# Opendigitalradio/ODR-AudioEnc

Measured on AMD Instinct MI355X. Metric: real-time stereo DAB MP2 streams sustained (frames/s) @128 kbps/48 kHz, higher is better.
Workload: dtype f64; 1 GPU; 4096 streams/GPU x 48 kHz stereo (mode 's') x 128 kbps, psy 1, full encode (BASELINE configs[1]), 32 frames/stream/step; streams_per_gpu=4096, parallelism=streams sharded over 1 GPU(s), no data-path collective

## Files before the change

### odr-audioenc_amd/csrc/mp2_fb.h

```cpp
#ifndef MP2_WAVE_PARTS
#error "include mp2_wave.h"
#endif
TL_FN void tl_filterbank(TlMainLds &w, const TlBlockShared *TL_RESTRICT B, const double *TL_RESTRICT enw_s, const int nch, PARGA(double, smp, 36))
{
    constexpr int FB = TlMainLds::kFbBatch;
        PA(int, xa, 16); PA(int, xb, 16);
        TL_LANES_BEGIN
        const int c = lane & 1, i = lane >> 1;
        const int ya = i == 0 ? 16 : i + 16, yb = i == 0 ? 16 : (i <= 16 ? 16 - i : 80 - i);
        for (int b = 0; b < 2; b++)
            for (int j = 1; j < 8; j++) {
                L(xa)[8 * b + ((0 - j) & 7)] = c < nch ? w.u.fbk.pcm[c][TL_HIST + 32 * b + 31 - ya - 64 * j] : 0;
                L(xb)[8 * b + ((0 - j) & 7)] = c < nch ? w.u.fbk.pcm[c][TL_HIST + 32 * b + 31 - yb - 64 * j] : 0;
            }
        TL_LANES_END
        TlMainLds::YpRows yp = w.yp;
#pragma unroll
        for (int b0 = 0; b0 < 36; b0 += FB) {
            TL_LANES_BEGIN
            const int c = lane & 1, i = lane >> 1;
            if (c < nch) {
                const int ya = i == 0 ? 16 : i + 16, yb = i == 0 ? 16 : (i <= 16 ? 16 - i : 80 - i);
                const uint64_t keep = i == 0 ? 0ull : ~0ull, flip = (i == 0 || i > 16) ? 0x8000000000000000ull : 0ull;
                int na[FB], nb[FB];
                double cf[8], ta[FB];
#pragma unroll
                for (int bb = 0; bb < FB; bb++) {
                    na[bb] = w.u.fbk.pcm[c][TL_HIST + 32 * (b0 + bb) + 31 - ya];
                    nb[bb] = w.u.fbk.pcm[c][TL_HIST + 32 * (b0 + bb) + 31 - yb];
                }
#pragma unroll
                for (int j = 0; j < 8; j++) cf[j] = enw_s[ya + 64 * j];
#pragma unroll
                for (int bb = 0; bb < FB; bb++) { TL_KEEP(na[bb]); TL_KEEP(nb[bb]); }
#pragma unroll
                for (int bb = 0; bb < FB; bb++) {
                    const int b = b0 + bb, q = 8 * (b & 1), h = b >> 1;
                    L(xa)[q + (h & 7)] = na[bb];
                    double t = (double)L(xa)[q + (h & 7)] * cf[0];
                    for (int j = 1; j < 8; j++) t += (double)L(xa)[q + ((h - j) & 7)] * cf[j];
                    ta[bb] = t;
                }
#pragma unroll
                for (int j = 0; j < 8; j++) cf[j] = enw_s[yb + 64 * j];
#pragma unroll
                for (int bb = 0; bb < FB; bb++) {
                    const int b = b0 + bb, q = 8 * (b & 1), h = b >> 1;
                    L(xb)[q + (h & 7)] = nb[bb];
                    double t = (double)L(xb)[q + (h & 7)] * cf[0];
                    for (int j = 1; j < 8; j++) t += (double)L(xb)[q + ((h - j) & 7)] * cf[j];
                    yp[bb][TL_YP_ROW * (2 * c + (i & 1)) + (i >> 1)] = ta[bb] + tl_u2d((tl_d2u(t) & keep) ^ flip);
                }
            }
            TL_LANES_END
            PA(double, part, FB);
            TL_LANES_BEGIN
            const int c = lane & 1, sb = lane >> 1, par = sb < 16 ? 0 : 1, r = sb < 16 ? sb : 31 - sb;
            double acc[FB];
            for (int bb = 0; bb < FB; bb++) acc[bb] = 0.0;
            if (c < nch)
                for (int k = 0; k < 16; k += 2) {
                    const double m0 = B->dct_t[k][par][r], m1 = B->dct_t[k + 1][par][r];
                    for (int bb = 0; bb < FB; bb++) {
                        double y0, y1;
                        TL_LD2(&yp[bb][TL_YP_ROW * (2 * c + par) + k], y0, y1);
                        acc[bb] += m0 * y0;
                        acc[bb] += m1 * y1;
                    }
                }
            for (int bb = 0; bb < FB; bb++) L(part)[bb] = acc[bb];
            TL_LANES_END
            PA(double, oth, FB);
            TL_MIRROR_SB_F64(oth, part, FB);
            TL_LANES_BEGIN
            const int sb = lane >> 1;
            if (sb < 16) { for (int bb = 0; bb < FB; bb++) L(smp)[b0 + bb] = L(part)[bb] + L(oth)[bb]; }
            else { for (int bb = 0; bb < FB; bb++) L(smp)[b0 + bb] = L(oth)[bb] - L(part)[bb]; }
            TL_LANES_END
        }
}
```

### odr-audioenc_amd/csrc/mp2_pack.h

```cpp
#ifndef MP2_WAVE_PARTS
#error "include mp2_wave.h"
#endif
struct TlFrameOut { uint8_t *bytes; uint32_t *words; uint8_t *scfcrc; };
template <int PSY, int NCH = 0>
TL_FN void tl_encode_frame(TlMainLds &w, const TlTables *TL_RESTRICT T, const TlBlockShared *TL_RESTRICT B,
                           const TlConfig *TL_RESTRICT C, const TlPsyOut *TL_RESTRICT PO,
                           const TlPcmView &pv, int xpad_len, const TlFrameOut &fo,
                           const double *TL_RESTRICT enw_s, const TlPackTables *TL_RESTRICT K, int padding, TlTaps *taps, long long *sp)
{
    constexpr int FB = TlMainLds::kFbBatch;
    const int nch = NCH ? NCH : C->nch, sblimit = C->sblimit;
    PA(double, smp, 36);
    PA(int, scf, 3);

    TL_STAMP(sp, 0);
    TL_PRIO2(TL_PS_FB);
    tl_filterbank(w, B, enw_s, nch, smp);

    TL_STAMP(sp, 1);
    TL_PRIO2(1);
#if !defined(TL_EMULATE) && TL_ENC_LEVEL >= 5
    for (int b = 0; b < 36; b++) TL_KEEP(smp[b]);
    scf[0] = scf[1] = scf[2] = 0;
#endif
    PV(int, a_ln); PV(int, a_nbal);
    TL_LANES_BEGIN
    {
        const int c = lane & 1, sb = lane >> 1;
        const bool live = c < nch && sb < sblimit;
        L(a_ln) = live ? C->line[sb] : 0;
        L(a_nbal) = live ? C->nbal[sb] : 0;
    }
    TL_LANES_END
    TL_LANES_BEGIN
    const int c = lane & 1, sb = lane >> 1;
    if (TL_ENC_LEVEL >= 5) { }
    else if (c < nch && sb < sblimit) {
        unsigned lo = 63;
        for (int gr = 0; gr < 3; gr++) {
            double m = fabs(L(smp)[gr * 12 + 11]);
            for (int j = 10; j >= 0; j--) { double t = fabs(L(smp)[gr * 12 + j]); if (t > m) m = t; }
            unsigned idx = tl_sf_index(B->scalefactor, m);
            L(scf)[gr] = (int)idx;
            w.scf[c][gr][sb] = (uint8_t)idx;
            if (idx < lo) lo = idx;
        }
        w.minidx[c][sb] = (uint8_t)lo;
    } else {
        L(scf)[0] = L(scf)[1] = L(scf)[2] = 0;
        if (sb >= sblimit || c >= nch) { w.minidx[c][sb] = 63; w.scf[c][0][sb] = w.scf[c][1][sb] = w.scf[c][2][sb] = 0; }
    }
    TL_LANES_END

    if (TL_ENC_LEVEL < 5 && C->mode0 == 1) {
        for (int gr = 0; gr < 3; gr++) {
            PV(double, jm);
            TL_LANES_BEGIN L(jm) = 0.0; TL_LANES_END
#pragma unroll
            for (int j = 11; j >= 0; j--) {
                PV(double, other);
                TL_SWAP1_F64(other, , smp, [gr * 12 + j]);
                TL_LANES_BEGIN
                double t = fabs(.5 * (L(smp)[gr * 12 + j] + L(other)));
                if (j == 11 || t > L(jm)) L(jm) = t;
                TL_LANES_END
            }
            TL_LANES_BEGIN
            const int c = lane & 1, sb = lane >> 1;
            if (c == 0 && sb < sblimit) w.jscale[gr][sb] = (uint8_t)tl_sf_index(B->scalefactor, L(jm));
            TL_LANES_END
        }
    }

    if (taps) {
        TL_LANES_BEGIN
        const int c = lane & 1, sb = lane >> 1;
        for (int b = 0; b < 36; b++) taps->sb_sample[c][b / 12][b % 12][sb] = L(smp)[b];
        for (int gr = 0; gr < 3; gr++) { taps->scalar_pre[c][gr][sb] = w.scf[c][gr][sb]; if (c == 0) taps->j_scale[gr][sb] = C->mode0 == 1 && sb < sblimit ? w.jscale[gr][sb] : 0; }
        taps->max_sc[c][sb] = (c < nch && sb < sblimit) ? B->scalefactor[w.minidx[c][sb]] : 1E-20;
        TL_LANES_END
    }

    TL_STAMP(sp, 2);
    if constexpr (TL_ENC_LEVEL >= 5) { }
    else if constexpr (PSY == 0) {
        TL_LANES_BEGIN
        const int c = lane & 1, sb = lane >> 1;
        if (c < nch) {
            int m = sb < sblimit ? (int)w.minidx[c][sb] : 0;
            w.smr[c][sb] = 2.0 * (30.0 - m) - C->p0_athmin[sb];
        }
        TL_LANES_END
    } else if constexpr (PSY == 2) {
        TL_LANES_BEGIN
        const int c = lane & 1, sb = lane >> 1;
        if (c < nch) w.smr[c][sb] = PO->a[c][sb];
        TL_LANES_END
    } else {
        static_assert(PSY == TL_PSY_EXT, "models 1 and 3");
        TL_LANES_BEGIN
        const int c = lane & 1, sb = lane >> 1;
        if (c < nch) {
            const double a = w.smr[c][sb], m = w.psy_m[c][sb];
            const double val = B->scale_db[w.minidx[c][sb]];
            const double top = a > val ? a : val;
            w.smr[c][sb] = top - m;
        }
        TL_LANES_END
    }

    TL_STAMP(sp, 3);
    TL_LANES_BEGIN
    const int c = lane & 1, sb = lane >> 1;
    if (TL_ENC_LEVEL < 5 && c < nch && sb < sblimit) {
        int s0 = L(scf)[0], s1 = L(scf)[1], s2 = L(scf)[2];
        int d0 = s0 - s1, d1 = s1 - s2;
        int c0 = d0 <= -3 ? 0 : d0 < 0 ? 1 : d0 == 0 ? 2 : d0 < 3 ? 3 : 4;
        int c1 = d1 <= -3 ? 0 : d1 < 0 ? 1 : d1 == 0 ? 2 : d1 < 3 ? 3 : 4;
        const unsigned p = B->sfpat[c0 * 5 + c1];
        const int m02 = s0 > s2 ? s2 : s0;
        const unsigned q0 = p & 3u, q1 = (p >> 2) & 3u, q2 = (p >> 4) & 3u;
        const int n0 = q0 == 0 ? s0 : q0 == 1 ? s1 : q0 == 2 ? s2 : m02;
        const int n1 = q1 == 0 ? s0 : q1 == 1 ? s1 : q1 == 2 ? s2 : m02;
        const int n2 = q2 == 0 ? s0 : q2 == 1 ? s1 : q2 == 2 ? s2 : m02;
        const int sel = (int)(p >> 6);
        s0 = n0; s1 = n1; s2 = n2;
        L(scf)[0] = s0; L(scf)[1] = s1; L(scf)[2] = s2;
        w.scf[c][0][sb] = (uint8_t)s0; w.scf[c][1][sb] = (uint8_t)s1; w.scf[c][2][sb] = (uint8_t)s2;
        w.scfsi[c][sb] = (uint8_t)sel;
    } else w.scfsi[c][sb] = 0;
    w.balloc[c][sb] = 0;
    TL_LANES_END

    const int lg_frame = C->frame_bytes + padding;
    int adb = lg_frame * 8 - (C->dab_ext * 8 + (xpad_len ? xpad_len : 2) * 8);
    int mode = C->mode0, mode_ext = C->mode_ext0, jsbound = C->jsbound0;
    PV(int, a_sfs); PV(int, a_sfs_o); PV(double, a_smr); PV(double, a_smr_o);
    TL_LANES_BEGIN
    const int c = lane & 1, sb = lane >> 1;
    const bool live = c < nch && sb < sblimit;
    L(a_sfs) = live ? 6 * tl_sfs_count(w.scfsi[c][sb]) : 0;
    L(a_sfs_o) = (live && nch == 2) ? 6 * tl_sfs_count(w.scfsi[1 - c][sb]) : 0;
    L(a_smr) = live ? w.smr[c][sb] : 0.0;
    L(a_smr_o) = (live && nch == 2) ? w.smr[1 - c][sb] : 0.0;
    TL_LANES_END
    if (TL_ENC_LEVEL < 4 && C->mode0 == 1) {
        PV(int, nz_own); PV(int, nz_jnt);
        TL_LANES_BEGIN
        int bo = 0, bj = 0;
        if (lane < 2 * sblimit) {
            const int ln = L(a_ln), maxAlloc = (1 << L(a_nbal)) - 1;
            double sv[15];
#pragma unroll
            for (int q = 0; q < 15; q++) sv[q] = B->snr_line[ln][q];
            int n1 = 0, n2 = 0;
#pragma unroll
            for (int q = 0; q < 15; q++) {
                const bool inr = q < maxAlloc - 1;
                n1 += (inr && !((sv[q] - L(a_smr)) >= 0.0)) ? 1 : 0;
                n2 += (inr && !((sv[q] - L(a_smr_o)) >= 0.0)) ? 1 : 0;
            }
            n2 = n2 > n1 ? n2 : n1;
            bo = n1 > 0 ? B->bits12_line[ln][n1] + 2 + L(a_sfs) : 0;
            bj = n2 > 0 ? B->bits12_line[ln][n2] + 4 + L(a_sfs) + L(a_sfs_o) : 0;
        }
        L(nz_own) = bo; L(nz_jnt) = bj;
        TL_LANES_END
        mode = 0; mode_ext = 0; jsbound = sblimit;
        int tries = 0, try_ext = 4;
        for (;;) {
// ... 186 lines not shown
                const bool three = L(q_grp) == 3;
                const unsigned M = (unsigned)L(q_steps);
                const unsigned fa = TL_SELECT(three, v[2], v[0]), fc = TL_SELECT(three, v[0], v[2]);
                const unsigned inner = v[1] + M * fc;
                tl_put_bits48(frame, pos, (uint64_t)fa + (uint64_t)M * (uint64_t)inner, L(q_grp) * nb);
            }
            if (taps) for (int x = 0; x < 3; x++) taps->subband[c][gr][j0 + x][sb] = (c < nch) ? v[x] : 0;
            TL_LANES_END
        }
        }
    }

    TL_STAMP(sp, 5);
    TL_PRIO2(1);
    unsigned crc16 = 0;
    if (TL_ENC_LEVEL < 1) {
    {
        const int n = 16 + (p_scf - 48);
        PV(uint32_t, part);
        TL_LANES_BEGIN
        uint32_t acc = 0;
        const bool preset = lane >= 62;
        const int first = 8 * lane;
        if (first < n || preset) {
            const int byte = lane < 2 ? lane + 2 : lane + 4;
            const int cnt = preset ? 8 : (n - first < 8 ? n - first : 8);
            const int e0 = preset ? n + 8 * (63 - lane) : 16 + (n - first - cnt);
            const uint16_t *xt = &K->crc_xpow[e0];
            const unsigned v = preset ? 0xffu : ((frame[byte >> 2] >> (24 - 8 * (byte & 3))) & 0xffu) >> (8 - cnt);
            unsigned x8[8];
#pragma unroll
            for (int k = 0; k < 8; k++) x8[k] = xt[k];
#pragma unroll
            for (int k = 0; k < 8; k++) acc ^= (0u - ((v >> k) & 1u)) & x8[k];
        }
        L(part) = acc;
        TL_LANES_END
        crc16 = TL_WAVE_XOR_U32(part) & 0xffffu;
    }
    const int tail = lg_frame - 2 - C->dab_ext;
    PV(int, rlen); PV(uint32_t, rcrc);
    TL_LANES_BEGIN
    const int c = lane & 1, sb = lane >> 1;
    uint32_t rec = 0;
    if (c < nch && sb < sblimit && w.balloc[c][sb]) {
        const uint32_t s0 = (uint32_t)L(scf)[0] >> 3, s1 = (uint32_t)L(scf)[1] >> 3, s2 = (uint32_t)L(scf)[2] >> 3;
        switch (w.scfsi[c][sb]) {
        case 0: rec = (9u << 16) | (s0 << 6) | (s1 << 3) | s2; break;
        case 1: case 3: rec = (6u << 16) | (s0 << 3) | s2; break;
        default: rec = (3u << 16) | s0; break;
        }
    }
    if (lane == 0) tl_put_bits(frame, 32, crc16, 16);
    L(rlen) = (int)(rec >> 16); L(rcrc) = rec & 0x1ffu;
    TL_LANES_END
    {
        PV(int, lex);
        TL_WAVE_EXSCAN_I32(lex, rlen);
        const int f[5] = {0, 4, 8, 16, 30};
        int gend[4], gfirst[4], glast[4];
        for (int g = 0; g < 4; g++) {
            gfirst[g] = f[g]; glast[g] = f[g + 1] > sblimit ? sblimit : f[g + 1];
            const int e = 2 * glast[g];
            gend[g] = (g < C->dab_ext && glast[g] > gfirst[g]) ? TL_READLANE_I32(lex, e) : 0;
        }
        PV(uint32_t, part); PV(uint32_t, pscan);
        TL_LANES_BEGIN
        const int sb = lane >> 1;
        const int g = sb < 4 ? 0 : sb < 8 ? 1 : sb < 16 ? 2 : 3;
        const int after = (g == 0 ? gend[0] : g == 1 ? gend[1] : g == 2 ? gend[2] : gend[3]) - L(lex) - L(rlen);
        const int e0 = after + 8;
        unsigned xp = K->crc8_xpow[e0 < 0 ? 0 : e0 > 319 ? 319 : e0];
        unsigned acc = 0;
        const unsigned rb = L(rcrc);
#pragma unroll
        for (int b = 0; b < 9; b++) {
            acc ^= ((rb >> b) & 1u) ? xp : 0u;
            xp = ((xp << 1) & 0xffu) ^ ((xp & 0x80u) ? 0x1Du : 0u);
        }
        L(part) = (L(rlen) && sb < sblimit) ? acc : 0u;
        TL_LANES_END
        TL_WAVE_INCL_XSCAN_U32(pscan, part);
        unsigned c8g[4];
        for (int g = 0; g < 4; g++) {
            c8g[g] = 0;
            if (g < C->dab_ext && glast[g] > gfirst[g]) {
                c8g[g] = (unsigned)TL_READLANE_I32(pscan, 2 * glast[g] - 1);
                if (gfirst[g] > 0) c8g[g] ^= (unsigned)TL_READLANE_I32(pscan, 2 * gfirst[g] - 1);
            }
        }
        TL_LANES_BEGIN
        if (lane < C->dab_ext) {
            const int grp = C->dab_ext - 1 - lane;
            const unsigned c8 = (grp == 0 ? c8g[0] : grp == 1 ? c8g[1] : grp == 2 ? c8g[2] : c8g[3]) & 0xffu;
            tl_put_bits(frame, (tail + lane) * 8, c8, 8);
            w.ncentre[lane] = (int16_t)c8;
        }
        TL_LANES_END
    }
    TL_LANES_BEGIN
    if (xpad_len) {
        const int xstart = lg_frame - C->dab_ext - xpad_len;
        for (int i = lane; i < xpad_len; i += 64) {
            int bytepos = i < xpad_len - 2 ? xstart + i : lg_frame - 2 + (i - (xpad_len - 2));
            tl_put_bits(frame, bytepos * 8, w.xpad[i], 8);
        }
    }
    TL_LANES_END

    } else {
        TL_LANES_BEGIN
        if (lane < 4) w.ncentre[lane] = 0;
        TL_LANES_END
    }
    if (taps) {
        TL_LANES_BEGIN
        const int c = lane & 1, sb = lane >> 1;
        taps->smr[c][sb] = (c < nch && (C->psy != 1 || sb < sblimit)) ? w.smr[c][sb] : 0.0;
        taps->scfsi[c][sb] = w.scfsi[c][sb]; taps->bit_alloc[c][sb] = w.balloc[c][sb];
        for (int gr = 0; gr < 3; gr++) taps->scalar[c][gr][sb] = w.scf[c][gr][sb];
        if (lane == 0) { taps->adb_left = adb_left; taps->mode = mode; taps->mode_ext = mode_ext; taps->jsbound = jsbound; taps->crc16 = (int)crc16; }
        if (lane < 4) taps->scfcrc[lane] = lane < C->dab_ext ? (uint8_t)w.ncentre[lane] : 0;
        TL_LANES_END
    }

    TL_STAMP(sp, 6);
    const int nwords = (lg_frame + 3) >> 2;
    TL_LANES_BEGIN
    for (int i = lane; i < nwords; i += 64) {
        if (fo.words) fo.words[i] = frame[i];
        else {
            const uint32_t le = tl_bswap(frame[i]);
            const int rem = lg_frame - 4 * i;
            if (rem >= 4) ((uint32_t *)fo.bytes)[i] = le;
            else for (int b = 0; b < rem; b++) fo.bytes[4 * i + b] = (uint8_t)(le >> (8 * b));
        }
    }
    if (lane < 4) fo.scfcrc[lane] = lane < C->dab_ext ? (uint8_t)w.ncentre[lane] : 0;
    TL_LANES_END
    TL_PRIO2(0);
    TL_STAMP(sp, 7);
}

template <int PSY>
TL_FN void tl_encode_pair(TlMainLds &w, const TlBlockShared *TL_RESTRICT B, const TlConfig *TL_RESTRICT C, const TlPsyOut *const (&PO)[2],
                          const int (&xpad_len)[2], const uint8_t *const (&xpad_src)[2], const TlFrameOut (&fo)[2],
                          const double *TL_RESTRICT enw_s, const TlPackTables *TL_RESTRICT K, const int (&padding)[2])
{
    const int sblimit = C->sblimit;
    const int padpk = padding[0] | (padding[1] << 1);
    PA(double, smp, 36);
    PA(int, scf, 3);
    TL_PRIO2(TL_PS_FB);
    tl_filterbank(w, B, enw_s, 2, smp);
    TL_PRIO2(1);
    TL_LANES_BEGIN
    const int c = lane & 1, sb = lane >> 1;
    if (sb < sblimit) {
        unsigned lo = 63;
        for (int gr = 0; gr < 3; gr++) {
            double m = fabs(L(smp)[gr * 12 + 11]);
            for (int j = 10; j >= 0; j--) { double t = fabs(L(smp)[gr * 12 + j]); if (t > m) m = t; }
            unsigned idx = tl_sf_index(B->scalefactor, m);
            L(scf)[gr] = (int)idx;
            if (idx < lo) lo = idx;
        }
        w.minidx[c][sb] = (uint8_t)lo;
    } else {
        L(scf)[0] = L(scf)[1] = L(scf)[2] = 0;
        w.minidx[c][sb] = 63;
    }
    TL_LANES_END
    TL_LANES_BEGIN
    const int c = lane & 1, sb = lane >> 1;
    if constexpr (PSY == 0) {
        const int m = sb < sblimit ? (int)w.minidx[c][sb] : 0;
        w.smr[c][sb] = 2.0 * (30.0 - m) - C->p0_athmin[sb];
    } else if constexpr (PSY == 2) {
        w.smr[c][sb] = (c ? PO[1] : PO[0])->a[0][sb];
    } else {
        const double a = w.smr[c][sb], m = w.psy_m[c][sb];
        const double val = B->scale_db[w.minidx[c][sb]];
        const double top = a > val ? a : val;
        w.smr[c][sb] = top - m;
    }
    TL_LANES_END
    TL_LANES_BEGIN
    const int c = lane & 1, sb = lane >> 1;
    if (sb < sblimit) {
        int s0 = L(scf)[0], s1 = L(scf)[1], s2 = L(scf)[2];
        int d0 = s0 - s1, d1 = s1 - s2;
        int c0 = d0 <= -3 ? 0 : d0 < 0 ? 1 : d0 == 0 ? 2 : d0 < 3 ? 3 : 4;
        int c1 = d1 <= -3 ? 0 : d1 < 0 ? 1 : d1 == 0 ? 2 : d1 < 3 ? 3 : 4;
        const unsigned p = B->sfpat[c0 * 5 + c1];
        const int m02 = s0 > s2 ? s2 : s0;
        const unsigned q0 = p & 3u, q1 = (p >> 2) & 3u, q2 = (p >> 4) & 3u;
        const int n0 = q0 == 0 ? s0 : q0 == 1 ? s1 : q0 == 2 ? s2 : m02;
        const int n1 = q1 == 0 ? s0 : q1 == 1 ? s1 : q1 == 2 ? s2 : m02;
        const int n2 = q2 == 0 ? s0 : q2 == 1 ? s1 : q2 == 2 ? s2 : m02;
        L(scf)[0] = n0; L(scf)[1] = n1; L(scf)[2] = n2;
        w.scfsi[c][sb] = (uint8_t)(p >> 6);
    } else w.scfsi[c][sb] = 0;
    w.balloc[c][sb] = 0;
    TL_LANES_END
    int lg_frame[2];
    {
        PV(int, a_ln); PV(int, a_nbal); PV(int, a_sfs); PV(double, a_smr); PV(int, ba);
        TL_LANES_BEGIN
        const int c = lane & 1, sb = lane >> 1;
        const bool live = sb < sblimit;
        L(a_ln) = live ? C->line[sb] : 0;
        L(a_nbal) = live ? C->nbal[sb] : 0;
        L(a_sfs) = live ? 6 * tl_sfs_count(w.scfsi[c][sb]) : 0;
        L(a_smr) = live ? w.smr[c][sb] : 0.0;
        TL_LANES_END
        int adb[2];
#pragma unroll
        for (int u = 0; u < 2; u++) {
            lg_frame[u] = C->frame_bytes + padding[u];
            adb[u] = lg_frame[u] * 8 - (C->dab_ext * 8 + (xpad_len[u] ? xpad_len[u] : 2) * 8);
        }
        tl_allocate_pair(B, adb[0], adb[1], sblimit, a_ln, a_nbal, a_sfs, a_smr, ba);
        TL_LANES_BEGIN
        const int c = lane & 1, sb = lane >> 1;
        w.balloc[c][sb] = (uint8_t)(sb < sblimit ? L(ba) : 0);
        TL_LANES_END
    }
    TL_LANES_BEGIN
    for (int i = lane; i < ((lg_frame[0] + 3) >> 2) + 2; i += 64) w.u.frame[0][i] = 0;
    for (int i = lane; i < ((lg_frame[1] + 3) >> 2) + 2; i += 64) w.u.frame[1][i] = 0;
    TL_LANES_END
    PV(int, f_ba); PV(int, f_sel); PV(int, f_scf); PV(int, f_smp); PV(int, a_ln2);
    PV(int, o_ba); PV(int, o_sel); PV(int, o_scf); PV(int, o_smp);
    TL_LANES_BEGIN
    const int c = lane & 1, sb = lane >> 1;
    const bool live = sb < sblimit;
    const int ba = live ? w.balloc[c][sb] : 0, sh = 16 * c;
    L(a_ln2) = live ? C->line[sb] : 0;
    L(f_ba) = (live ? (int)C->nbal[sb] : 0) << sh;
    L(f_sel) = (ba ? 2 : 0) << sh;
    L(f_scf) = (ba ? 6 * tl_sfs_count(w.scfsi[c][sb]) : 0) << sh;
    L(f_smp) = (ba ? B->bits12_line[L(a_ln2)][ba] / 12 : 0) << sh;
    TL_LANES_END
    TL_WAVE_EXSCAN_I32(o_ba, f_ba); TL_WAVE_EXSCAN_I32(o_sel, f_sel);
    TL_WAVE_EXSCAN_I32(o_scf, f_scf); TL_WAVE_EXSCAN_I32(o_smp, f_smp);
    const int s_ba = TL_WAVE_SUM_I32(f_ba), s_sel = TL_WAVE_SUM_I32(f_sel), s_scf = TL_WAVE_SUM_I32(f_scf), s_smp = TL_WAVE_SUM_I32(f_smp);
    int p_sel[2], p_scf[2], p_smp[2], n_smp[2];
#pragma unroll
    for (int u = 0; u < 2; u++) {
        const int sh = 16 * u;
        p_sel[u] = 48 + ((s_ba >> sh) & 0xffff); p_scf[u] = p_sel[u] + ((s_sel >> sh) & 0xffff); p_smp[u] = p_scf[u] + ((s_scf >> sh) & 0xffff);
        n_smp[u] = (s_smp >> sh) & 0xffff;
    }
    TL_LANES_BEGIN
    const int c = lane & 1, sb = lane >> 1, sh = 16 * c;
    uint32_t *frame = w.u.frame[c];
    if (lane < 2) {
        uint32_t h = (0xfffu << 20) | ((uint32_t)C->version << 19) | (2u << 17) | (0u << 16)
                   | ((uint32_t)C->br_idx << 12) | ((uint32_t)C->fs_idx << 10) | ((uint32_t)((padpk >> c) & 1) << 9) | (0u << 8)
                   | ((uint32_t)C->mode0 << 6) | ((uint32_t)C->mode_ext0 << 4);
        TL_ATOMIC_OR(&frame[0], h);
    }
    const bool live = sb < sblimit;
    const int ba = live ? w.balloc[c][sb] : 0;
    const int nb_ba = (L(f_ba) >> sh) & 0xffff;
    if (nb_ba) tl_put_bits48(frame, 48 + ((L(o_ba) >> sh) & 0xffff), (uint64_t)ba, nb_ba);
    if (ba) {
        const unsigned si = w.scfsi[c][sb];
        tl_put_bits48(frame, (c ? p_sel[1] : p_sel[0]) + ((L(o_sel) >> sh) & 0xffff), si, 2);
        const unsigned s0 = (unsigned)L(scf)[0], s1 = (unsigned)L(scf)[1], s2 = (unsigned)L(scf)[2];
        const unsigned f3 = (s0 << 12) | (s1 << 6) | s2, f2 = (s0 << 6) | s2;
        tl_put_bits48(frame, (c ? p_scf[1] : p_scf[0]) + ((L(o_scf) >> sh) & 0xffff), si == 0 ? f3 : si == 2 ? s0 : f2, (L(f_scf) >> sh) & 0xffff);
    }
    TL_LANES_END
    TL_PRIO2(TL_PS_Q);
    {
        PV(int, q_ba); PV(int, q_nb); PV(int, q_grp); PV(int, q_s2n); PV(int, q_steps); PV(int, q_pos); PV(int, q_rstep);
        PV(double, q_a); PV(double, q_b); PV(double, q_s2nf); PA(double, q_sf, 3); PA(double, q_rsf, 3);
        TL_LANES_BEGIN
        const int c = lane & 1, sb = lane >> 1, sh = 16 * c;
        const int ba = sb < sblimit ? w.balloc[c][sb] : 0;
        const unsigned qi = ba ? B->qinfo_line[L(a_ln2)][ba] : 0u;
        const int q = (int)(qi & 31u);
        L(q_ba) = ba; L(q_nb) = (int)((qi >> 5) & 31u); L(q_grp) = ((qi >> 10) & 1u) ? 3 : 1; L(q_s2n) = K->steps2n[q];
        L(q_steps) = ((qi >> 10) & 1u) ? 1 << L(q_nb) : K->steps[q];
        L(q_a) = K->qa[q]; L(q_b) = K->qb[q]; L(q_s2nf) = K->steps2n_f[q];
        for (int gr = 0; gr < 3; gr++) {
            L(q_sf)[gr] = B->scalefactor[L(scf)[gr]];
            L(q_rsf)[gr] = 1.0 / L(q_sf)[gr];
        }
        L(q_pos) = (c ? p_smp[1] : p_smp[0]) + ((L(o_smp) >> sh) & 0xffff);
        L(q_rstep) = c ? n_smp[1] : n_smp[0];
        TL_LANES_END
#pragma unroll
        for (int r = 0; r < 12; r++) {
            const int gr = r >> 2, j0 = (r & 3) * 3;
            TL_LANES_BEGIN
            if (L(q_ba)) {
                const double sfv = L(q_sf)[gr], rsf = L(q_rsf)[gr];
                unsigned v[3];
                for (int x = 0; x < 3; x++) {
                    double d = tl_div_by(L(smp)[gr * 12 + j0 + x], sfv, rsf);
                    d = d * L(q_a) + L(q_b);
                    const bool neg = !(d >= 0);
                    d += TL_SELECT(neg, 1.0, 0.0);
                    const unsigned qv = (unsigned)(d * L(q_s2nf));
                    v[x] = qv | (neg ? 0u : (unsigned)L(q_s2n));
// ... 130 lines not shown
```

### odr-audioenc_amd/csrc/mp2_wave.h

```cpp
#pragma once
#include "mp2_types.h"
#include "tl_libm.h"
#include <math.h>
#include <stddef.h>

#ifdef TL_EMULATE
#define TL_FN static inline
#define TL_LANES_BEGIN for (int lane = 0; lane < 64; ++lane) {
#define TL_LANES_END }
#define TL_SYNC() ((void)0)
#define PV(T, name) T name[64]
#define PA(T, name, n) T name[64][n]
#define L(name) name[lane]
#define PARG(T, name) T (&name)[64]
#define PARGA(T, name, n) T (&name)[64][n]
#define TL_OTHER(name, idx, src) name[src] idx
#define TL_ATOMIC_OR(p, v) (*(p) |= (v))
TL_FN uint64_t tlh_ballot(const bool (&p)[64]) { uint64_t m = 0; for (int i = 0; i < 64; i++) if (p[i]) m |= 1ull << i; return m; }
TL_FN uint64_t tlh_min_u64(const uint64_t (&v)[64]) { uint64_t m = v[0]; for (int i = 1; i < 64; i++) if (v[i] < m) m = v[i]; return m; }
TL_FN int tlh_sum_i32(const int (&v)[64]) { int s = 0; for (int i = 0; i < 64; i++) s += v[i]; return s; }
TL_FN uint32_t tlh_xor_u32(const uint32_t (&v)[64]) { uint32_t s = 0; for (int i = 0; i < 64; i++) s ^= v[i]; return s; }
TL_FN void tlh_exscan_i32(int (&d)[64], const int (&v)[64]) { int s = 0; for (int i = 0; i < 64; i++) { d[i] = s; s += v[i]; } }
TL_FN int tlh_argmin_u64(const uint64_t (&v)[64])
{
// ... 108 lines not shown
}
TL_FN double tld_row16_max_f64(double v)
{
    double o;
    o = tld_row_shr_f64<1>(v); v = v < o ? o : v;
    o = tld_row_shr_f64<2>(v); v = v < o ? o : v;
    o = tld_row_shr_f64<4>(v); v = v < o ? o : v;
    o = tld_row_shr_f64<8>(v); v = v < o ? o : v;
    return v;
}
#define TL_ROW16_MAX_F64(dst, src) dst = tld_row16_max_f64(src)
TL_FN uint32_t tld_par_min_u32(uint32_t v)
{
    uint32_t t;
    t = (uint32_t)__builtin_amdgcn_update_dpp((int)v, (int)v, 0x122, 0xf, 0xf, false); v = t < v ? t : v;
    t = (uint32_t)__builtin_amdgcn_update_dpp((int)v, (int)v, 0x124, 0xf, 0xf, false); v = t < v ? t : v;
    t = (uint32_t)__builtin_amdgcn_update_dpp((int)v, (int)v, 0x128, 0xf, 0xf, false); v = t < v ? t : v;
    const auto r = __builtin_amdgcn_permlane16_swap(v, v, false, false); v = r[0] < r[1] ? r[0] : r[1];
    const auto q = __builtin_amdgcn_permlane32_swap(v, v, false, false); v = q[0] < q[1] ? q[0] : q[1];
    return v;
}
TL_FN uint64_t tld_par_min_u64(uint64_t v)
{
    const uint32_t hi = (uint32_t)(v >> 32), lo = (uint32_t)v;
    const uint32_t mhi = tld_par_min_u32(hi);
    const uint32_t mlo = tld_par_min_u32(hi == mhi ? lo : 0xffffffffu);
    return ((uint64_t)mhi << 32) | mlo;
}
TL_FN int tld_par_sum_i32(int v)
{
    v += __builtin_amdgcn_update_dpp(v, v, 0x122, 0xf, 0xf, false);
    v += __builtin_amdgcn_update_dpp(v, v, 0x124, 0xf, 0xf, false);
    v += __builtin_amdgcn_update_dpp(v, v, 0x128, 0xf, 0xf, false);
    const auto r = __builtin_amdgcn_permlane16_swap((unsigned)v, (unsigned)v, false, false); v = (int)(r[0] + r[1]);
    const auto q = __builtin_amdgcn_permlane32_swap((unsigned)v, (unsigned)v, false, false); v = (int)(q[0] + q[1]);
    return v;
}
#define TL_PAR_MIN_U64(dst, src) dst = tld_par_min_u64(src)
#define TL_PAR_SUM_I32(dst, src) dst = tld_par_sum_i32(src)
#define TL_BALLOT(name) ((uint64_t)__ballot(name))
#define TL_SWAP1_U64(dst, src) dst = tl_d2u(tld_swap1_f64(tl_u2d(src)))
#define TL_SWAP1_F64(dst, di, src, si) dst di = tld_swap1_f64(src si)
#define TL_SPLAT(dst, di, val) dst di = (val)
#define TL_ROT32_F64(dst, src) dst = __shfl(src, (int)((threadIdx.x + 32u) & 63u), 64)
#define TL_MIRROR_SB_F64(dst, src, n) do { const int lane_ = (int)(threadIdx.x & 63u), partner_ = 2 * (31 - (lane_ >> 1)) + (lane_ & 1); \
                                           _Pragma("unroll") for (int k_ = 0; k_ < (n); k_++) dst[k_] = __shfl(src[k_], partner_, 64); } while (0)
#define TL_WAVE_ARGMIN_U64(name) tld_argmin_u64(name)
#define TL_WAVE_MIN_U64(name) tld_min_u64(name)
#define TL_WAVE_SUM_I32(name) tld_sum_i32(name)
#define TL_WAVE_XOR_U32(name) tld_xor_u32(name)
#define TL_WAVE_EXSCAN_I32(dst, src) dst = tld_exscan_i32(src)
#define TL_UNI_I(x) __builtin_amdgcn_readfirstlane(x)
#define TL_READLANE_I32(name, l) __builtin_amdgcn_readlane(name, l)
#define TL_RESTRICT __restrict__
#define TL_SELECT(c, a, b) (__builtin_unpredictable(c) ? (a) : (b))
#define TL_KEEP(x) asm volatile("" : : "v"(x))
typedef double tl_f64x2 __attribute__((ext_vector_type(2)));
#define TL_LD2(p, a, b) do { const tl_f64x2 v_ = *(const tl_f64x2 *)(p); (a) = v_.x; (b) = v_.y; } while (0)
#define TL_ST2(p, a, b) do { tl_f64x2 v_; v_.x = (a); v_.y = (b); *(tl_f64x2 *)(p) = v_; } while (0)
#define TL_RANK_BELOW(mask) ((int)__builtin_amdgcn_mbcnt_hi((uint32_t)((mask) >> 32), __builtin_amdgcn_mbcnt_lo((uint32_t)(mask), 0u)))
#if defined(__HIP_DEVICE_COMPILE__)
typedef const __attribute__((address_space(4))) struct TlLaunch *TlKArg;
#else
typedef const struct TlLaunch *TlKArg;
#endif
#define TL_KARG TlKArg
#define TL_LAUNDER(p) asm volatile("" : "+s"(p))
#define TL_TIE(p, v) asm volatile("" : "+s"(p), "+v"(v))
TL_FN int tl_sign_bit(double x) { int r; asm("v_lshrrev_b32 %0, 31, %1" : "=v"(r) : "v"((uint32_t)(tl_d2u(x) >> 32))); return r; }
#define TL_SCHED_FENCE() __builtin_amdgcn_sched_barrier(0)
#define TL_SCT(t, row, j) ((t)[((row) >> 1) + ((j) & 1) + 220 * ((j) >> 1)])
#define TL_PIN(x) asm volatile("" : "+v"(x))
#endif

#ifndef TL_PRIO_CHAIN
#define TL_PRIO_CHAIN 3
#endif
#ifndef TL_PS_FHT
#define TL_PS_FHT 0
#endif
#ifndef TL_PS_THR
#define TL_PS_THR 1
#endif
#ifndef TL_PS_FB
#define TL_PS_FB 0
#endif
#ifndef TL_PS_Q
#define TL_PS_Q 0
#endif
#ifndef TL_PS_POW
#define TL_PS_POW 1
#endif
#ifndef TL_PRIO_SERIAL
#define TL_PRIO_SERIAL 2
#endif
#ifdef TL_EMULATE
#define TL_PRIO(n) ((void)0)
#define TL_PRIO2(n) ((void)0)
#else
#define TL_PRIO(n) do { if (TL_PRIO_CHAIN) __builtin_amdgcn_s_setprio((n) ? TL_PRIO_CHAIN : TL_PRIO_SERIAL); } while (0)
#define TL_PRIO2(n) do { if (TL_PRIO_SERIAL) __builtin_amdgcn_s_setprio((n) ? TL_PRIO_SERIAL : 0); } while (0)
#endif
#ifdef TL_EMULATE
#define TL_STAMP(sp, k) ((void)0)
#else
#define TL_STAMP(sp, k) do { if (sp) { long long t_ = (long long)__builtin_amdgcn_s_memtime(); if ((threadIdx.x & 63u) == 0) (sp)[k] = t_; } } while (0)
#endif

#if defined(TL_EMULATE) && defined(TL_DEBUG_DUMP)
#include <stdio.h>
#include <stdlib.h>
#define TL_DBG_DUMP(tag, ch, nt, nn, x, b) do { if (getenv("TL_DUMP")) { printf("%s ch%d ntone %d nnoise %d:", tag, ch, nt, nn); \
    for (int i_ = 0; i_ < (nt) + (nn); i_++) printf(" (%.17g,%.6f)", (x)[i_], (b)[i_]); printf("\n"); } } while (0)
#define TL_DBG_WALK(ch, lane, cnt) do { if (getenv("TL_DUMP_WALK")) printf("walk ch%d lane %d cnt %d\n", ch, lane, cnt); } while (0)
static long tl_dbg_rounds = 0, tl_dbg_tones = 0, tl_dbg_deadheads = 0, tl_dbg_fronts = 0, tl_dbg_cands = 0;
#define TL_DBG_CAND(n) (tl_dbg_cands += (n))
#define TL_DBG_ROUND() (tl_dbg_rounds++)
#define TL_DBG_TONES(n, dh) (tl_dbg_tones += (n), tl_dbg_deadheads += (dh) ? 1 : 0, tl_dbg_fronts++)
static long tl_dbg_back[7] = {0, 0, 0, 0, 0, 0, 0};
#define TL_DBG_BACK(k) (tl_dbg_back[k]++)
extern "C" __attribute__((weak, visibility("default"))) void emu_back_stats(long *out) { for (int i = 0; i < 7; i++) out[i] = tl_dbg_back[i]; }
#else
#define TL_DBG_BACK(k) ((void)0)
#define TL_DBG_DUMP(tag, ch, nt, nn, x, b) ((void)0)
#define TL_DBG_WALK(ch, lane, cnt) ((void)0)
#define TL_DBG_ROUND() ((void)0)
#define TL_DBG_TONES(n, dh) ((void)0)
#define TL_DBG_CAND(n) ((void)0)
#endif
#ifndef TL_EXP_LEVEL
#define TL_EXP_LEVEL 0
#endif
#ifndef TL_ENC_LEVEL
#define TL_ENC_LEVEL 0
#endif
#ifndef TL_P2_LEVEL
#define TL_P2_LEVEL 0
#endif
#ifndef TL_P2_SUB
#define TL_P2_SUB 0
#endif
#ifndef TL_P3_NOTAIL
#define TL_P3_NOTAIL 0
#endif
#define TL_DBMIN (-200.0)
#define TL_POWERNORM 90.3090
#define TL_T_NOISE 10
#define TL_T_TONE 20
#define TL_LAST (-1)
#define TL_STOP (-100)

#define TL_CAND_MAX 256
#ifndef TL_FB_BATCH_MAIN
#define TL_FB_BATCH_MAIN 6
#endif
#define TL_PSY_EXT 5
#define TL_TONE_MAX 77
#define TL_MASKER_MAX 128
#define TL_FFT_WORDS (513 + 520)
#define TL_PX(w) ((w).u.fft + 513)
#define TL_EX(i) ((i) ^ (((i) >> 4) & 15))
#define TL_YP_ROW 18
struct TlMainLds {
    static constexpr int kFbBatch = TL_FB_BATCH_MAIN;
    union alignas(16) {
        struct { int16_t pcm[2][TL_HIST + 1152]; } fbk;
        uint32_t frame[2][TL_MAX_FRAME_WORDS + 2];
    } u;
    alignas(16) double yp[TL_FB_BATCH_MAIN][TL_YP_ROW * 3 + 16];
    double smr[2][32];
    double psy_m[2][32];
    int16_t ncentre[32];
    uint8_t scf[2][3][32];
    uint8_t jscale[3][32];
    uint8_t scfsi[2][32];
    uint8_t balloc[2][32];
    uint8_t minidx[2][32];
    uint8_t xpad[TL_MAX_XPAD];
    typedef double (*YpRows)[TL_YP_ROW * 3 + 16];
};
#ifndef TL_Q_REDEAL
#define TL_Q_REDEAL 1
#endif
#ifndef TL_Q_REDEAL_MAX
#define TL_Q_REDEAL_MAX 48
#endif
struct alignas(16) TlQCell { double a, b, s2nf; uint32_t w0, w1; };
struct alignas(16) TlQGran { double s[12]; double sf, rsf; };
#define TL_QRD_OFF ((4 * (TL_MAX_FRAME_WORDS + 2) + 15) & ~15)
#define TL_QRD_CELLS(w) ((TlQCell *)((char *)&(w) + TL_QRD_OFF))
#define TL_QRD_GRANS(w) ((TlQGran *)((char *)&(w) + TL_QRD_OFF + TL_Q_REDEAL_MAX * sizeof(TlQCell)))
static_assert(sizeof(TlQCell) == 32 && sizeof(TlQGran) == 112, "records are whole 16-byte pieces");
static_assert(offsetof(TlMainLds, u) == 0 && offsetof(TlMainLds, yp) == sizeof(((TlMainLds *)0)->u) && offsetof(TlMainLds, yp) % 16 == 0,
              "yp[] follows the staging union without a gap");
static_assert(TL_QRD_OFF + TL_Q_REDEAL_MAX * (sizeof(TlQCell) + sizeof(TlQGran)) <= offsetof(TlMainLds, yp) + sizeof(((TlMainLds *)0)->yp),
              "cell records and granule blocks end inside yp[]");
static_assert(TL_Q_REDEAL_MAX >= 0 && TL_Q_REDEAL_MAX <= 64 && TL_MAX_FRAME_BYTES * 8 / 12 < (1 << 11), "a rank per lane; o_smp fits its 11 bits");
struct alignas(16) TlPsy2Lds {
    struct { double fft[1024]; } u;
    double px[536];
};
struct TlPsyLds {
    struct { double fft[TL_FFT_WORDS]; } u;
    double tone_x[TL_TONE_MAX];
    double nsum[32];
    uint32_t cinfo[TL_CAND_MAX];
    int16_t conf_c[TL_TONE_MAX];
    int16_t conf_nxt[TL_TONE_MAX];
    int16_t tlist[TL_TONE_MAX];
    int16_t ncentre[32];
    int16_t bandoff[40];
    uint8_t ptype[520];
};
#define TL_MK_X(w) ((w).u.fft)
#define TL_MK_BARK(w) ((w).u.fft + TL_MASKER_MAX)
#define TL_LTG(w) ((w).u.fft + 2 * TL_MASKER_MAX)
struct TlMasker { double bark, av, g, c17, n; };
#define TL_MK4(w) ((TlMasker *)((w).u.fft + 2 * TL_MASKER_MAX + 136))
static_assert(2 * TL_MASKER_MAX + 136 + 5 * TL_MASKER_MAX <= TL_FFT_WORDS, "masker records fit the transform buffer");
#define TL_P1B_LIST 32
#define TL_P1B_BASE 700
#define TL_P1B_MKX(w) ((w).u.fft + TL_P1B_BASE)
#define TL_P1B_MKBARK(w) ((w).u.fft + TL_P1B_BASE + 64)
#define TL_P1B_TONE_X(w) ((w).u.fft + TL_P1B_BASE + 128)
#define TL_P1B_PTYPE(w) ((uint8_t *)((w).u.fft + TL_P1B_BASE + 128 + TL_TONE_MAX))
#define TL_P1B_CONF_C(w) ((int16_t *)((w).u.fft + TL_P1B_BASE + 128 + TL_TONE_MAX + 65))
static_assert(TL_P1B_LIST + 27 <= 64 && 2 * TL_MASKER_MAX + 136 + 5 * (TL_P1B_LIST + 27) <= TL_P1B_BASE, "channel 1's masker records end below channel 0's records");
static_assert(TL_P1B_BASE + 128 + TL_TONE_MAX + 65 + (2 * TL_TONE_MAX + 7) / 8 <= TL_FFT_WORDS, "channel 0's records fit the transform buffer");



#ifdef TL_EMULATE
static long tl_emu_near1_full = 0;
#define TL_DBG_NEAR1_FULL() (tl_emu_near1_full++)
#else
#define TL_DBG_NEAR1_FULL() ((void)0)
#endif
#ifdef TL_EMULATE
static long tl_emu_redeal[2][66];
#define TL_DBG_REDEAL(took, ba) do { int n_ = 0; for (int l_ = 0; l_ < 64; l_++) n_ += (ba)[l_] != 0; \
                                     tl_emu_redeal[(took) ? 1 : 0][0]++; tl_emu_redeal[(took) ? 1 : 0][1 + n_]++; } while (0)
extern "C" __attribute__((weak, visibility("default"))) void emu_redeal_stats(long *out)
{ out[0] = tl_emu_redeal[0][0]; out[1] = tl_emu_redeal[1][0]; for (int i = 0; i < 65; i++) { out[2 + i] = tl_emu_redeal[0][1 + i]; out[67 + i] = tl_emu_redeal[1][1 + i]; } }
#else
#define TL_DBG_REDEAL(took, ba) ((void)0)
#endif

#define MP2_WAVE_PARTS 1
#include "mp2_dbsum.h"
#include "mp2_fht.h"
#include "mp2_psy13.h"
#include "mp2_psy24.h"
#include "mp2_fb.h"
#include "mp2_alloc.h"
#include "mp2_pack.h"
#include "mp2_units.h"
#undef MP2_WAVE_PARTS
```

Baseline: 36.99 million frames/s.

## Raise main filterbank batch to nine by overlaying extra rows on PCM staging

The filterbank batch size becomes a template parameter. The main encode path now processes 9 blocks per batch instead of 6, while the PSY_EXT frame path keeps 6. The three extra matrixing row blocks are placed in the already-consumed low part of the PCM history staging area, so the LDS footprint does not grow. Static asserts check that these rows do not clobber samples still to be read and that the four rows of each read land on distinct banks. Fewer batch iterations mean fewer barriers and mirror exchanges, at the cost of more registers per lane.

```diff
diff --git a/odr-audioenc_amd/csrc/mp2_fb.h b/odr-audioenc_amd/csrc/mp2_fb.h
--- a/odr-audioenc_amd/csrc/mp2_fb.h
+++ b/odr-audioenc_amd/csrc/mp2_fb.h
@@ -1,9 +1,10 @@
 #ifndef MP2_WAVE_PARTS
 #error "include mp2_wave.h"
 #endif
+template <int FB>
 TL_FN void tl_filterbank(TlMainLds &w, const TlBlockShared *TL_RESTRICT B, const double *TL_RESTRICT enw_s, const int nch, PARGA(double, smp, 36))
 {
-    constexpr int FB = TlMainLds::kFbBatch;
+    static_assert(FB >= 1 && FB <= TlMainLds::kFbBatchMax && 36 % FB == 0, "a batch size the LDS block was laid out for");
         PA(int, xa, 16); PA(int, xb, 16);
         TL_LANES_BEGIN
         const int c = lane & 1, i = lane >> 1;
@@ -14,7 +15,6 @@
                 L(xb)[8 * b + ((0 - j) & 7)] = c < nch ? w.u.fbk.pcm[c][TL_HIST + 32 * b + 31 - yb - 64 * j] : 0;
             }
         TL_LANES_END
-        TlMainLds::YpRows yp = w.yp;
 #pragma unroll
         for (int b0 = 0; b0 < 36; b0 += FB) {
             TL_LANES_BEGIN
@@ -49,7 +49,7 @@
                     L(xb)[q + (h & 7)] = nb[bb];
                     double t = (double)L(xb)[q + (h & 7)] * cf[0];
                     for (int j = 1; j < 8; j++) t += (double)L(xb)[q + ((h - j) & 7)] * cf[j];
-                    yp[bb][TL_YP_ROW * (2 * c + (i & 1)) + (i >> 1)] = ta[bb] + tl_u2d((tl_d2u(t) & keep) ^ flip);
+                    tl_fb_row(w, bb, c, i & 1)[i >> 1] = ta[bb] + tl_u2d((tl_d2u(t) & keep) ^ flip);
                 }
             }
             TL_LANES_END
@@ -63,7 +63,7 @@
                     const double m0 = B->dct_t[k][par][r], m1 = B->dct_t[k + 1][par][r];
                     for (int bb = 0; bb < FB; bb++) {
                         double y0, y1;
-                        TL_LD2(&yp[bb][TL_YP_ROW * (2 * c + par) + k], y0, y1);
+                        TL_LD2(tl_fb_row(w, bb, c, par) + k, y0, y1);
                         acc[bb] += m0 * y0;
                         acc[bb] += m1 * y1;
                     }
diff --git a/odr-audioenc_amd/csrc/mp2_pack.h b/odr-audioenc_amd/csrc/mp2_pack.h
--- a/odr-audioenc_amd/csrc/mp2_pack.h
+++ b/odr-audioenc_amd/csrc/mp2_pack.h
@@ -8,14 +8,13 @@
                            const TlPcmView &pv, int xpad_len, const TlFrameOut &fo,
                            const double *TL_RESTRICT enw_s, const TlPackTables *TL_RESTRICT K, int padding, TlTaps *taps, long long *sp)
 {
-    constexpr int FB = TlMainLds::kFbBatch;
     const int nch = NCH ? NCH : C->nch, sblimit = C->sblimit;
     PA(double, smp, 36);
     PA(int, scf, 3);
 
     TL_STAMP(sp, 0);
     TL_PRIO2(TL_PS_FB);
-    tl_filterbank(w, B, enw_s, nch, smp);
+    tl_filterbank<tl_fb_batch(PSY)>(w, B, enw_s, nch, smp);
 
     TL_STAMP(sp, 1);
     TL_PRIO2(1);
@@ -508,7 +507,7 @@
     PA(double, smp, 36);
     PA(int, scf, 3);
     TL_PRIO2(TL_PS_FB);
-    tl_filterbank(w, B, enw_s, 2, smp);
+    tl_filterbank<tl_fb_batch(PSY)>(w, B, enw_s, 2, smp);
     TL_PRIO2(1);
     TL_LANES_BEGIN
     const int c = lane & 1, sb = lane >> 1;
diff --git a/odr-audioenc_amd/csrc/mp2_wave.h b/odr-audioenc_amd/csrc/mp2_wave.h
--- a/odr-audioenc_amd/csrc/mp2_wave.h
+++ b/odr-audioenc_amd/csrc/mp2_wave.h
@@ -284,8 +284,13 @@
 
 #define TL_CAND_MAX 256
 #ifndef TL_FB_BATCH_MAIN
-#define TL_FB_BATCH_MAIN 6
-#endif
+#define TL_FB_BATCH_MAIN 9
+#endif
+#ifndef TL_FB_BATCH_FRAME
+#define TL_FB_BATCH_FRAME 6
+#endif
+#define TL_FB_BATCH_MAX (TL_FB_BATCH_MAIN > TL_FB_BATCH_FRAME ? TL_FB_BATCH_MAIN : TL_FB_BATCH_FRAME)
+#define TL_FB_YP_BLOCKS (TL_FB_BATCH_MAX < 6 ? TL_FB_BATCH_MAX : 6)
 #define TL_PSY_EXT 5
 #define TL_TONE_MAX 77
 #define TL_MASKER_MAX 128
@@ -293,13 +298,17 @@
 #define TL_PX(w) ((w).u.fft + 513)
 #define TL_EX(i) ((i) ^ (((i) >> 4) & 15))
 #define TL_YP_ROW 18
+#define TL_PCM_ROW_DOUBLES ((TL_HIST + 1152) / 4)
+#define TL_FB_OV_BLOCK (TL_YP_ROW + 16)
 struct TlMainLds {
-    static constexpr int kFbBatch = TL_FB_BATCH_MAIN;
+    static constexpr int kFbBatchMax = TL_FB_BATCH_MAX;
+    static constexpr int kFbYpBlocks = TL_FB_YP_BLOCKS;
     union alignas(16) {
         struct { int16_t pcm[2][TL_HIST + 1152]; } fbk;
+        double fbrow[2][TL_PCM_ROW_DOUBLES];
         uint32_t frame[2][TL_MAX_FRAME_WORDS + 2];
     } u;
-    alignas(16) double yp[TL_FB_BATCH_MAIN][TL_YP_ROW * 3 + 16];
+    alignas(16) double yp[TL_FB_YP_BLOCKS][TL_YP_ROW * 3 + 16];
     double smr[2][32];
     double psy_m[2][32];
     int16_t ncentre[32];
@@ -309,8 +318,34 @@
     uint8_t balloc[2][32];
     uint8_t minidx[2][32];
     uint8_t xpad[TL_MAX_XPAD];
-    typedef double (*YpRows)[TL_YP_ROW * 3 + 16];
+    static constexpr int fb_row_at(int bb, int c, int par, int yp_at)
+    { return bb < kFbYpBlocks ? yp_at + (TL_YP_ROW * 3 + 16) * bb + TL_YP_ROW * (2 * c + par) : TL_PCM_ROW_DOUBLES * c + TL_FB_OV_BLOCK * (bb - kFbYpBlocks) + TL_YP_ROW * par; }
+    static constexpr bool fb_rows_spread(int yp_at)
+    {
+        for (int bb = 0; bb < kFbBatchMax; bb++) {
+            int quad[4] = {0, 0, 0, 0};
+            for (int r = 0; r < 4; r++) {
+                const int at = fb_row_at(bb, r >> 1, r & 1, yp_at);
+                if (at % 2) return false;
+                quad[r] = (at / 2) % 16;
+            }
+            for (int r = 0; r < 4; r++) for (int q = 0; q < r; q++) if (quad[r] == quad[q]) return false;
+        }
+        return true;
+    }
 };
+TL_FN double *tl_fb_row(TlMainLds &w, int bb, int c, int par)
+{
+    if (bb < TlMainLds::kFbYpBlocks) return &w.yp[bb][TL_YP_ROW * (2 * c + par)];
+    return &w.u.fbrow[c][TL_FB_OV_BLOCK * (bb - TlMainLds::kFbYpBlocks) + TL_YP_ROW * par];
+}
+constexpr int tl_fb_batch(int psy) { return psy == TL_PSY_EXT ? TL_FB_BATCH_FRAME : TL_FB_BATCH_MAIN; }
+static_assert(sizeof(((TlMainLds *)0)->u.fbrow) == sizeof(((TlMainLds *)0)->u.fbk) && (TL_HIST + 1152) % 4 == 0 && (TL_PCM_ROW_DOUBLES * 8) % 16 == 0,
+              "the overlay is the staging area itself; both channels' regions start 16-byte aligned");
+static_assert(TL_FB_BATCH_MAIN >= 1 && 36 % TL_FB_BATCH_MAIN == 0 && TL_FB_BATCH_FRAME >= 1 && 36 % TL_FB_BATCH_FRAME == 0, "whole batches");
+static_assert(TL_HIST - 32 >= 0 && (TL_FB_BATCH_MAX - TL_FB_YP_BLOCKS) * TL_FB_OV_BLOCK * 4 <= TL_HIST - 32,
+              "a channel's overlay rows (4 samples to the double) end at or below the first sample the batches still read, TL_HIST - 32");
+static_assert(TL_FB_OV_BLOCK % 2 == 0 && (TL_YP_ROW * 3 + 16) % 2 == 0 && TL_YP_ROW % 2 == 0, "16-byte reads of a row's pairs stay aligned in every block");
 #ifndef TL_Q_REDEAL
 #define TL_Q_REDEAL 1
 #endif
@@ -325,6 +360,7 @@
 static_assert(sizeof(TlQCell) == 32 && sizeof(TlQGran) == 112, "records are whole 16-byte pieces");
 static_assert(offsetof(TlMainLds, u) == 0 && offsetof(TlMainLds, yp) == sizeof(((TlMainLds *)0)->u) && offsetof(TlMainLds, yp) % 16 == 0,
               "yp[] follows the staging union without a gap");
+static_assert(TlMainLds::fb_rows_spread((int)(offsetof(TlMainLds, yp) / 8)), "the four rows of a matrixing read fall on different banks, in yp[] and in the overlay");
 static_assert(TL_QRD_OFF + TL_Q_REDEAL_MAX * (sizeof(TlQCell) + sizeof(TlQGran)) <= offsetof(TlMainLds, yp) + sizeof(((TlMainLds *)0)->yp),
               "cell records and granule blocks end inside yp[]");
 static_assert(TL_Q_REDEAL_MAX >= 0 && TL_Q_REDEAL_MAX <= 64 && TL_MAX_FRAME_BYTES * 8 / 12 < (1 << 11), "a rank per lane; o_smp fits its 11 bits");
```

Result: no change. 36.96 million frames/s (-0.1%).
